# benabbouosama/DEEPL-Project

Hardware: AMD Instinct MI355X
Metric: images/sec train step, TransVAE-Large f16d32 256px bs256 (higher is better)
Workload: dtype bf16

## Files before the change

deepl-project_amd/csrc/wgrad_kx3.hip:

```cpp
#include "common.h"

#include <type_traits>

namespace {

struct Kx3Args {
    const bf16* x;
    const bf16* gy;
    float* dw;
    float* dbias;
    int M, h, w, c_in, ldx, c_out, ldo;
    int tiles_ci, chunk_px, hw_shift, w_shift, plain;
    int xcd_order, base, ny, accum;
    unsigned x_bytes;
};

template <int TW>
__device__ __forceinline__ int kx_swz(int c, int r) {
    if constexpr (TW % 128 == 0) {
        return (c & ~15) | ((c & 15) ^ ((r & 7) << 1));
    } else if constexpr (TW % 64 == 0) {
        return (c & ~7) | ((c & 7) ^ (((r >> 1) & 3) << 1));
    } else {
        static_assert(TW % 32 == 0, "tile width");
        return (c & ~3) | ((c & 3) ^ (((r >> 2) & 1) << 1));
    }
}

constexpr int kx_seg_stride(int seg) { return (seg + 2 + 7) / 8 * 8; }
constexpr int kx_x_pieces(int seg, int cx) { return ((64 / seg) * kx_seg_stride(seg) * cx + 63) / 64; }
constexpr int kx_stage_bytes(int tg, int tx, int seg) { return 64 * tg * 2 + kx_x_pieces(seg, tx / 8) * 1024; }

template <int TG, int TX, int NWM, int NWN, int RING, int VAR, int SEG, int TAPS = 3>
__global__ __launch_bounds__(512, 1) void wgrad_kx3_kernel(const Kx3Args p) {
    constexpr int NW = 8, BKP = 64;
    static_assert(NWM * NWN == NW, "8 waves");
    static_assert(SEG == 16 || SEG == 32 || SEG == 64, "segment = min(image width, 64)");
    static_assert(TAPS == 3 || (TAPS == 1 && SEG == 64), "one tap: 64 consecutive rows per K-step");
    constexpr int CG = TG / 8, CX = TX / 8;
    constexpr int NSEG = BKP / SEG, SS = TAPS == 1 ? 64 : kx_seg_stride(SEG);
    constexpr int G_PIECES = BKP * CG / 64;
    constexpr int X_PIECES = TAPS == 1 ? CX : kx_x_pieces(SEG, CX);
    static_assert(G_PIECES % NW == 0, "gy pieces divide over the waves");
    constexpr int G_IT = G_PIECES / NW, X_IT = (X_PIECES + NW - 1) / NW, P_IT = G_IT + X_IT;
    constexpr int XR = X_PIECES % NW;
    constexpr int G_BYTES = BKP * TG * 2, X_BYTES = X_PIECES * 1024;
    constexpr int KK_ROWS = SEG == 64 ? 32 : (32 / SEG) * SS, H_ROWS = SEG == 16 ? SS : 16;
    constexpr int X_REGION = RING * G_BYTES;
    static_assert(RING * (G_BYTES + X_BYTES) <= 160 * 1024, "LDS");
    constexpr int WTG = TG / NWM, WTX = TX / NWN, MF = WTG / 16, NF = WTX / 16;
    static_assert(WTG % 16 == 0 && WTX % 16 == 0, "wave tile");
    constexpr bool RD_SPLIT = VAR == 1 || VAR == 2 || VAR == 3;
    constexpr int LOOK = (VAR == 2 || VAR == 3) ? RING - 2 : RING - 1;
    constexpr int IT_SPLIT = VAR == 1 ? 0 : ((VAR == 2 || VAR == 4) ? G_IT : P_IT);
    static_assert(LOOK >= 2, "the wait at the end of load phase t covers K-step t + 1");

    extern __shared__ __attribute__((aligned(16))) char smem[];
    const int tid = threadIdx.x, lane = tid & 63;
    const int wave = __builtin_amdgcn_readfirstlane(tid >> 6);
    const int wm = wave / NWN, wn = wave % NWN;

    int bx, chunk_id;
    if (p.xcd_order) {
        const int lin = blockIdx.x;
        const int xcd = lin & 7, j = lin >> 3;
        bx = j % p.base;
        chunk_id = (j / p.base) * 8 + xcd;
        if (chunk_id >= p.ny) return;
    } else {
        bx = blockIdx.x;
        chunk_id = blockIdx.y;
    }
    const int ci_tile = bx % p.tiles_ci;
    bx /= p.tiles_ci;
    const int ky = TAPS == 3 ? bx % 3 : 0;
    const int co_tile = TAPS == 3 ? bx / 3 : bx;
    const int co0 = co_tile * TG, ci0 = ci_tile * TX;
    const int p_begin = chunk_id * p.chunk_px;
    const int p_end = min(p.M, p_begin + p.chunk_px);
    const int nsteps = (p_end - p_begin) / BKP;
    if (nsteps <= 0) return;
    const int w = p.w, hw = p.h * p.w;
    const int dty = TAPS == 3 ? ky - 1 : 0;

    int g_voff[G_IT];
#pragma unroll
    for (int it = 0; it < G_IT; ++it) {
        const int id = (it * NW + wave) * 64 + lane;
        const int r = id / CG, sl = id - r * CG;
        g_voff[it] = (r * p.ldo + co0 + kx_swz<TG>(sl, r) * 8) * 2;
    }
    int x_voff[X_IT], x_need[X_IT];
#pragma unroll
    for (int it = 0; it < X_IT; ++it) {
        const int id = (it * NW + wave) * 64 + lane;
        const int R = id / CX, sl = id - R * CX;
        const int sg = R / SS, o = R - sg * SS;
        const int need = TAPS == 1 ? 1 : (o == 0 ? 2 : (o == SEG + 1 ? 4 : (o > SEG + 1 ? 0 : 1)));
        x_need[it] = sg < NSEG ? need << (3 * sg) : 0;
        x_voff[it] = ((sg * SEG + o) * p.ldx + ci0 + kx_swz<TX>(sl, R) * 8) * 2;
    }
    const long long dshift = TAPS == 1 ? 0 : ((long long)dty * w - 1) * p.ldx;
    const bf16* xb = p.x + dshift;
    const unsigned xb_bytes = (unsigned)((long long)p.x_bytes - dshift * 2);
    const unsigned g_bytes = (unsigned)((long long)p_end * p.ldo * 2);

    auto x_have = [&](int step) {
        int have = 0;
        if constexpr (TAPS == 1) return 1;
#pragma unroll
        for (int sg = 0; sg < NSEG; ++sg) {
            const int pz = p_begin + step * BKP + sg * SEG;
            const int x0 = pz & (w - 1);
            const int uy = ((pz & (hw - 1)) >> p.w_shift) + dty;
            if ((unsigned)uy < (unsigned)p.h) have |= (1 | (x0 != 0 ? 2 : 0) | (x0 + SEG < w ? 4 : 0)) << (3 * sg);
        }
        return have;
    };
    auto issue_piece = [&](auto it_c, int step, int slot, int have) {
        constexpr int IT = decltype(it_c)::value;
        const int pz = p_begin + step * BKP;
        if constexpr (IT < G_IT) {
            buffer_load_lds16(p.gy, g_bytes, smem + slot * G_BYTES + (IT * NW + wave) * 1024, g_voff[IT], pz * p.ldo * 2);
        } else {
            constexpr int XI = IT - G_IT;
            if (XR != 0 && XI == X_IT - 1 && wave >= XR) return;
            buffer_load_lds16(xb, xb_bytes, smem + X_REGION + slot * X_BYTES + (XI * NW + wave) * 1024,
                              (x_need[XI] & have) ? x_voff[XI] : OOB_OFFSET, pz * p.ldx * 2);
        }
    };
    auto stage_issue = [&](int step, int slot) {
        const int have = x_have(step);
        static_for<P_IT>([&](auto it_c) { issue_piece(it_c, step, slot, have); });
    };

    const int g = lane >> 4, q = (lane >> 2) & 3, pp = lane & 3;
    const unsigned smem_addr = (unsigned)(uintptr_t)(__attribute__((address_space(3))) char*)smem;
    unsigned a_base[MF];
#pragma unroll
    for (int i = 0; i < MF; ++i) {
        const int r = 4 * g + q;
        const int col = wm * WTG + i * 16 + 4 * pp;
        a_base[i] = smem_addr + r * (TG * 2) + kx_swz<TG>(col >> 3, r) * 16 + (pp & 1) * 8;
    }
    unsigned b_base[TAPS][NF];
#pragma unroll
    for (int tp = 0; tp < TAPS; ++tp) {
        const int R = 4 * g + q + tp;
#pragma unroll
        for (int j = 0; j < NF; ++j) {
            const int col = wn * WTX + j * 16 + 4 * pp;
            b_base[tp][j] = smem_addr + X_REGION + R * (TX * 2) + kx_swz<TX>(col >> 3, R) * 16 + (pp & 1) * 8;
        }
    }
    constexpr int A_IN = 32 * TG * 2 + 16 * TG * 2, B_IN = (KK_ROWS + H_ROWS) * TX * 2;
    constexpr bool A_TWO = (RING - 1) * G_BYTES + A_IN >= 65536, B_TWO = (RING - 1) * X_BYTES + B_IN >= 65536;
    static_assert(!A_TWO || ((RING - 3) * G_BYTES + A_IN < 65536 && G_BYTES + A_IN < 65536), "gy slot offsets");
    static_assert(!B_TWO || ((RING - 3) * X_BYTES + B_IN < 65536 && X_BYTES + B_IN < 65536), "x slot offsets");
    unsigned a_base2[MF], b_base2[TAPS][NF];
#pragma unroll
    for (int i = 0; i < MF; ++i) a_base2[i] = a_base[i] + (A_TWO ? 2 * G_BYTES : 0);
#pragma unroll
    for (int tp = 0; tp < TAPS; ++tp)
#pragma unroll
        for (int j = 0; j < NF; ++j) b_base2[tp][j] = b_base[tp][j] + (B_TWO ? 2 * X_BYTES : 0);

    f32x4 acc[TAPS][MF][NF];
#pragma unroll
    for (int tp = 0; tp < TAPS; ++tp)
#pragma unroll
        for (int i = 0; i < MF; ++i)
#pragma unroll
            for (int j = 0; j < NF; ++j) acc[tp][i][j] = f32x4{0.f, 0.f, 0.f, 0.f};

    const bool do_bias = p.dbias != nullptr;
    const int nshare = TAPS * p.tiles_ci;
    int bias_ctr = ky * p.tiles_ci + ci_tile;
    bool own = false, own_prev = false;
    constexpr int NB = (MF + NWN - 1) / NWN;
    float bsum[NB];
#pragma unroll
    for (int k = 0; k < NB; ++k) bsum[k] = 0.f;

    auto join = [](bf16x4 lo, bf16x4 hi) { return bf16x8{lo[0], lo[1], lo[2], lo[3], hi[0], hi[1], hi[2], hi[3]}; };
    bf16x4 alo[2][MF], ahi[2][MF], blo[2][TAPS][NF], bhi[2][TAPS][NF];
    const int grp = wave >> 2;

    constexpr int NR = 2 * MF + 2 * TAPS * NF, NM = TAPS * MF * NF;
    auto frag_read = [&](auto kk_c, auto r_c, auto slot_c) {
        constexpr int KK = decltype(kk_c)::value, R = decltype(r_c)::value, SLOT = decltype(slot_c)::value;
        if constexpr (R < 2 * MF) {
            constexpr int i = R / 2, h = R % 2;
            constexpr int OFF = ((A_TWO && SLOT >= 2) ? (SLOT - 2) * G_BYTES : SLOT * G_BYTES) + KK * 32 * TG * 2 + h * 16 * TG * 2;
            const unsigned ab = (A_TWO && SLOT >= 2) ? a_base2[i] : a_base[i];
            if constexpr (h == 0) alo[KK][i] = lds_tr16_imm<OFF>(ab);
            else ahi[KK][i] = lds_tr16_imm<OFF>(ab);
        } else {
            constexpr int rr = R - 2 * MF, tp = rr / (2 * NF), j = (rr / 2) % NF, h = rr % 2;
            constexpr int OFF = ((B_TWO && SLOT >= 2) ? (SLOT - 2) * X_BYTES : SLOT * X_BYTES) + KK * KK_ROWS * TX * 2 + h * H_ROWS * TX * 2;
            const unsigned bb = (B_TWO && SLOT >= 2) ? b_base2[tp][j] : b_base[tp][j];
            if constexpr (h == 0) blo[KK][tp][j] = lds_tr16_imm<OFF>(bb);
            else bhi[KK][tp][j] = lds_tr16_imm<OFF>(bb);
        }
    };
    auto mfma_one = [&](auto kk_c, auto m_c) {
        constexpr int KK = decltype(kk_c)::value, M = decltype(m_c)::value;
        constexpr int i = M / (TAPS * NF), tp = (M / NF) % TAPS, j = M % NF;
        acc[tp][i][j] = __builtin_amdgcn_mfma_f32_16x16x32_bf16(join(alo[KK][i], ahi[KK][i]), join(blo[KK][tp][j], bhi[KK][tp][j]), acc[tp][i][j], 0, 0, 0);
    };
    auto bias_add = [&](auto kk_c) {
        constexpr int KK = decltype(kk_c)::value;
#pragma unroll
        for (int i = 0; i < MF; ++i)
            if (i % NWN == wn) {
                float a = 0.f;
#pragma unroll
                for (int e = 0; e < 4; ++e) a += (float)alo[KK][i][e] + (float)ahi[KK][i][e];
                bsum[i / NWN] += a;
            }
    };
    using I0 = std::integral_constant<int, 0>;
    using I1 = std::integral_constant<int, 1>;

#pragma unroll
    for (int st = 0; st < LOOK; ++st)
        if (st < nsteps) stage_issue(st, st);
    wait_vmcnt<0>();
    if (grp == 1) __builtin_amdgcn_s_barrier();

    auto step = [&](int t, auto slot_c) {
        constexpr int SLOT = decltype(slot_c)::value;
        constexpr int FILL = (SLOT + LOOK) % RING;
        const bool more = t + LOOK < nsteps;
        own_prev = own;
        own = do_bias && bias_ctr == 0;
        bias_ctr = bias_ctr == 0 ? nshare - 1 : bias_ctr - 1;
        __builtin_amdgcn_s_barrier();
        if constexpr (RD_SPLIT) {
            if (own_prev) bias_add(I1{});
            __builtin_amdgcn_sched_barrier(0);
        }
        static_for<NR>([&](auto r_c) { frag_read(I0{}, r_c, slot_c); });
        if constexpr (!RD_SPLIT) static_for<NR>([&](auto r_c) { frag_read(I1{}, r_c, slot_c); });
        __builtin_amdgcn_sched_barrier(0);
        const int have = more ? x_have(t + LOOK) : 0;
        if (more) static_for<IT_SPLIT>([&](auto it_c) { issue_piece(it_c, t + LOOK, FILL, have); });
        __builtin_amdgcn_sched_barrier(0);
        asm volatile("s_waitcnt lgkmcnt(0)" ::: "memory");
        __builtin_amdgcn_sched_barrier(0);
        if (own) {
            bias_add(I0{});
            if constexpr (!RD_SPLIT) bias_add(I1{});
        }
        {
            constexpr int NLG = IT_SPLIT < G_IT ? IT_SPLIT : G_IT;
            constexpr int NLX = IT_SPLIT > G_IT ? IT_SPLIT - G_IT : 0;
            constexpr int P_HI = G_IT + X_IT, P_LO = G_IT + X_IT - (XR != 0 ? 1 : 0);
            constexpr int L_HI = NLG + NLX, L_LO = NLG + NLX - ((XR != 0 && NLX == X_IT) ? 1 : 0);
            if (!more) wait_vmcnt<0>();
            else if (XR != 0 && wave < XR) wait_vmcnt<(LOOK - 2) * P_HI + L_HI>();
            else wait_vmcnt<(LOOK - 2) * P_LO + L_LO>();
        }
        __builtin_amdgcn_s_barrier();
        __builtin_amdgcn_s_setprio(1);
        if constexpr (!RD_SPLIT && IT_SPLIT == P_IT) {
            static_for<NM>([&](auto m_c) { mfma_one(I0{}, m_c); });
            static_for<NM>([&](auto m_c) { mfma_one(I1{}, m_c); });
        } else {
            constexpr int NP = P_IT - IT_SPLIT;
            static_for<NM>([&](auto m_c) {
                constexpr int M = decltype(m_c)::value;
                mfma_one(I0{}, m_c);
                __builtin_amdgcn_sched_barrier(0);
                if constexpr (RD_SPLIT) {
                    constexpr int r0 = M * NR / NM, r1 = (M + 1) * NR / NM;
                    static_for<r1 - r0>([&](auto d_c) { frag_read(I1{}, std::integral_constant<int, r0 + decltype(d_c)::value>{}, slot_c); });
                }
                if constexpr (NP > 0) {
                    static_for<NP>([&](auto k_c) {
                        constexpr int K = decltype(k_c)::value;
                        if constexpr ((2 * K + 1) * 2 * NM / (2 * NP) == M) {
                            if (more) issue_piece(std::integral_constant<int, IT_SPLIT + K>{}, t + LOOK, FILL, have);
                        }
                    });
                }
                __builtin_amdgcn_sched_barrier(0);
            });
            if constexpr (RD_SPLIT) {
                asm volatile("s_waitcnt lgkmcnt(0)" ::: "memory");
                __builtin_amdgcn_sched_barrier(0);
            }
            static_for<NM>([&](auto m_c) {
                constexpr int M = decltype(m_c)::value + NM;
                mfma_one(I1{}, m_c);
                if constexpr (NP > 0) {
                    __builtin_amdgcn_sched_barrier(0);
                    static_for<NP>([&](auto k_c) {
                        constexpr int K = decltype(k_c)::value;
                        if constexpr ((2 * K + 1) * 2 * NM / (2 * NP) == M) {
                            if (more) issue_piece(std::integral_constant<int, IT_SPLIT + K>{}, t + LOOK, FILL, have);
                        }
                    });
                    __builtin_amdgcn_sched_barrier(0);
                }
            });
        }
        __builtin_amdgcn_s_setprio(0);
        __builtin_amdgcn_sched_barrier(0);
    };

    for (int t = 0; t < nsteps; t += RING) {
        step(t, std::integral_constant<int, 0>{});
        if (t + 1 < nsteps) step(t + 1, std::integral_constant<int, 1>{});
        if (t + 2 < nsteps) step(t + 2, std::integral_constant<int, 2 % RING>{});
        if constexpr (RING == 4) {
            if (t + 3 < nsteps) step(t + 3, std::integral_constant<int, 3 % RING>{});
        }
    }
    if constexpr (RD_SPLIT) {
        if (own) bias_add(I1{});
    }
    if (grp == 0) __builtin_amdgcn_s_barrier();

    const size_t ldw = (size_t)(TAPS * TAPS) * p.c_in;
#pragma unroll
    for (int i = 0; i < MF; ++i) {
#pragma unroll
        for (int r = 0; r < 4; ++r) {
            const int co = co0 + wm * WTG + i * 16 + g * 4 + r;
#pragma unroll
            for (int tp = 0; tp < TAPS; ++tp) {
                float* rowp = p.dw + (size_t)co * ldw + (size_t)(ky * TAPS + tp) * p.c_in;
#pragma unroll
                for (int j = 0; j < NF; ++j) {
                    const int ci = ci0 + wn * WTX + j * 16 + (lane & 15);
                    if (p.plain && !p.accum) rowp[ci] = acc[tp][i][j][r];
                    else if (p.plain) rowp[ci] += acc[tp][i][j][r];
                    else atomicAdd(rowp + ci, acc[tp][i][j][r]);
                }
            }
        }
    }
    if (do_bias) {
#pragma unroll
        for (int i = 0; i < MF; ++i)
            if (i % NWN == wn) {
                float v = bsum[i / NWN];
                v += __shfl_xor(v, 16, 64);
                v += __shfl_xor(v, 32, 64);
                const int co = co0 + wm * WTG + i * 16 + (lane & 15);
                if (lane < 16) atomicAdd(p.dbias + co, v);
            }
    }
}

int g_kx3_ring = 0;
int g_kx3_var = -1;
int g_kx3_blocks = 0;

template <int TG, int TX, int NWM, int NWN, int RING, int VAR, int SEG, int TAPS = 3>
int kx3_launch_v(const Kx3Args& a, dim3 grid, hipStream_t s) {
    constexpr int BYTES = RING * (TAPS == 1 ? 64 * (TG + TX) * 2 : kx_stage_bytes(TG, TX, SEG));
    static_assert(BYTES <= 160 * 1024, "LDS");
    static TvPerDeviceOnce attr_once;
    if (attr_once.first()) {
        (void)hipFuncSetAttribute((const void*)wgrad_kx3_kernel<TG, TX, NWM, NWN, RING, VAR, SEG, TAPS>, hipFuncAttributeMaxDynamicSharedMemorySize, BYTES);
    }
    hipLaunchKernelGGL((wgrad_kx3_kernel<TG, TX, NWM, NWN, RING, VAR, SEG, TAPS>), grid, dim3(512), BYTES, s, a);
    return 0;
}

template <int TG, int TX, int NWM, int NWN, int RING, int SEG, int TAPS = 3>
int kx3_launch_r(Kx3Args a, hipStream_t s, bool plan_only) {
    const int tiles_co = a.c_out / TG;
    a.tiles_ci = a.c_in / TX;
    const long long base = (long long)tiles_co * TAPS * a.tiles_ci;
    const double t_px = 2.0 * TG * TX * TAPS * 256.0 / 1200e12;
    const double tile_bytes = 4.0 * TG * TX * TAPS;
    long long split = 1;
    bool xcd = false;
    double best = 1e30;
    const long long smax = a.M / 512 > 0 ? a.M / 512 : 1;
    if (g_kx3_blocks) {
        split = (g_kx3_blocks + base - 1) / base;
        xcd = base <= 32 && split >= 8;
    } else {
        for (long long sp = 1; sp <= smax && sp <= 4096; ++sp) {
            const double rounds = (double)((long long)((base * sp + 255) / 256));
            const double t = rounds * ((double)a.M / sp) * t_px + (sp > 1 ? base * sp * tile_bytes / 1.3e12 : 0.0);
            if (t < best) { best = t; split = sp; xcd = false; }
        }
        if (base <= 32) {
            for (long long sp = 8; sp <= smax && sp <= 4096; sp += 8) {
                const double rounds = (double)((long long)((base * (sp / 8) + 31) / 32));
                const double t = rounds * ((double)a.M / sp) * (t_px * 0.85) + base * sp * tile_bytes / 1.3e12;
                if (t < best) { best = t; split = sp; xcd = true; }
            }
        }
    }
    long long chunk = (a.M + split - 1) / split;
    if (chunk < 512) chunk = 512;
    chunk = (chunk + 63) / 64 * 64;
    a.chunk_px = (int)chunk;
    const int ny = (int)((a.M + chunk - 1) / chunk);
    a.plain = (ny == 1) ? 1 : 0;
    if (plan_only) return 100 + a.plain;
    a.base = (int)base;
    a.ny = ny;
    a.xcd_order = (ny > 1 && xcd) ? 1 : 0;
    dim3 grid((unsigned)base, (unsigned)ny);
    if (a.xcd_order) grid = dim3((unsigned)(8 * base * ((ny + 7) / 8)), 1);
    if constexpr (TAPS == 1) {
        if (g_kx3_var == 0) return kx3_launch_v<TG, TX, NWM, NWN, RING, 0, SEG, 1>(a, grid, s);
        return kx3_launch_v<TG, TX, NWM, NWN, RING, 4, SEG, 1>(a, grid, s);
    } else if constexpr (RING == 4 && SEG == 64) {
        switch (g_kx3_var < 0 ? 4 : g_kx3_var) {
            case 1: return kx3_launch_v<TG, TX, NWM, NWN, RING, 1, SEG>(a, grid, s);
            case 2: return kx3_launch_v<TG, TX, NWM, NWN, RING, 2, SEG>(a, grid, s);
            case 3: return kx3_launch_v<TG, TX, NWM, NWN, RING, 3, SEG>(a, grid, s);
            case 4: return kx3_launch_v<TG, TX, NWM, NWN, RING, 4, SEG>(a, grid, s);
            default: break;
        }
    }
    if (g_kx3_var != 0) return kx3_launch_v<TG, TX, NWM, NWN, RING, 4, SEG>(a, grid, s);
    return kx3_launch_v<TG, TX, NWM, NWN, RING, 0, SEG>(a, grid, s);
}

template <int TG, int TX, int NWM, int NWN, int SEG>
int kx3_launch_s(const Kx3Args& a, hipStream_t s, bool plan_only) {
    if constexpr (4 * kx_stage_bytes(TG, TX, SEG) <= 160 * 1024) {
        if (g_kx3_ring != 3) return kx3_launch_r<TG, TX, NWM, NWN, 4, SEG>(a, s, plan_only);
    }
    return kx3_launch_r<TG, TX, NWM, NWN, 3, SEG>(a, s, plan_only);
}

template <int TG, int TX, int NWM, int NWN>
int kx3_launch(const Kx3Args& a, hipStream_t s, bool plan_only) {
    if (a.w >= 64) return kx3_launch_s<TG, TX, NWM, NWN, 64>(a, s, plan_only);
    if (a.w == 32) return kx3_launch_s<TG, TX, NWM, NWN, 32>(a, s, plan_only);
    return kx3_launch_s<TG, TX, NWM, NWN, 16>(a, s, plan_only);
}

}

extern "C" int tv_set_wgrad_kx3(int enable, int ring, int blocks);
int g_kx3_enable = 2;
int g_kx3_prefer128 = 0;
extern "C" int tv_set_wgrad_kx3(int enable, int ring, int blocks) {
    g_kx3_enable = enable;
    g_kx3_ring = ring % 10;
    g_kx3_var = ring >= 10 ? ring / 10 : (ring == 0 ? -1 : 0);
    g_kx3_blocks = blocks % 100000;
    g_kx3_prefer128 = blocks / 100000;
    return 0;
}

int tv_wgrad_kx3_try(const tv_conv_desc* d, const void* x, const void* gy, float* dw, float* dbias, hipStream_t s, bool plan_only, int accum) {
    if (!g_kx3_enable) return -1;
    auto log2_exact = [](int v) { int sh = 0; while ((1 << sh) < v) ++sh; return ((1 << sh) == v) ? sh : -1; };
    if (d->kh == 1 && d->kw == 1) {
        const long long Ml = (long long)d->batch * d->h_out * d->w_out;
        const bool ok = g_kx3_enable % 10 >= 2 && d->stride == 1 && d->pad == 0 && d->up_shift == 0 && d->dil_mask == 0 && d->h_in == d->h_out &&
                        d->w_in == d->w_out && Ml % 64 == 0 && Ml * d->ldx * 2 < (1ll << 31) && Ml * d->ldo * 2 < (1ll << 31) &&
                        d->c_out % 192 == 0 && d->c_in % 192 == 0;
        if (!ok) return -1;
        Kx3Args a;
        a.x = (const bf16*)x; a.gy = (const bf16*)gy; a.dw = dw; a.dbias = dbias;
        a.M = (int)Ml; a.h = 1; a.w = 64; a.c_in = d->c_in; a.ldx = d->ldx; a.c_out = d->c_out; a.ldo = d->ldo;
        a.tiles_ci = 1; a.chunk_px = 0; a.hw_shift = 6; a.w_shift = 6; a.plain = 0;
        a.xcd_order = 0; a.base = 1; a.ny = 1; a.accum = accum;
        a.x_bytes = (unsigned)(Ml * d->ldx * 2);
        const int tsel = g_kx3_enable / 10;
        if (tsel == 1 && d->c_out % 256 == 0 && d->c_in % 128 == 0) return kx3_launch_r<256, 128, 4, 2, 3, 64, 1>(a, s, plan_only);
        if (tsel == 2 && d->c_out % 128 == 0 && d->c_in % 256 == 0) return kx3_launch_r<128, 256, 2, 4, 3, 64, 1>(a, s, plan_only);
        return kx3_launch_r<192, 192, 4, 2, 3, 64, 1>(a, s, plan_only);
    }
    const int wsh = log2_exact(d->w_out), hwsh = log2_exact(d->h_out * d->w_out);
    const long long M = (long long)d->batch * d->h_out * d->w_out;
    const long long xbytes = M * d->ldx * 2, gbytes = M * d->ldo * 2;
    const bool geo = d->kh == 3 && d->kw == 3 && d->stride == 1 && d->pad == 1 && d->up_shift == 0 && d->dil_mask == 0 &&
                     d->h_in == d->h_out && d->w_in == d->w_out && wsh >= 4 && hwsh >= 6 &&
                     xbytes + (long long)(d->w_in + 1) * d->ldx * 2 < (1ll << 31) && gbytes < (1ll << 31);
    if (!geo) return -1;
    const bool t192 = d->c_out % 192 == 0 && d->c_in % 96 == 0;
    const bool t128 = d->c_out % 128 == 0 && d->c_in % 128 == 0;
    if (!t192 && !t128) return -1;
    Kx3Args a;
    a.x = (const bf16*)x; a.gy = (const bf16*)gy; a.dw = dw; a.dbias = dbias;
    a.M = (int)M; a.h = d->h_out; a.w = d->w_out; a.c_in = d->c_in; a.ldx = d->ldx; a.c_out = d->c_out; a.ldo = d->ldo;
    a.tiles_ci = 1; a.chunk_px = 0; a.hw_shift = hwsh; a.w_shift = wsh; a.plain = 0;
    a.xcd_order = 0; a.base = 1; a.ny = 1; a.accum = accum;
    a.x_bytes = (unsigned)xbytes;
    if (t192 && !(t128 && g_kx3_prefer128 != 2)) return kx3_launch<192, 96, 4, 2>(a, s, plan_only);
    return kx3_launch<128, 128, 2, 4>(a, s, plan_only);
}
```

Before: 160.6.

## Add wide 384x192 tiles with 32-row K-steps for 1x1 weight-gradient kernel

After: 161.5 (median of 6 runs). Within noise of the previous version (+0.6%).

```diff
diff --git a/deepl-project_amd/csrc/wgrad_kx3.hip b/deepl-project_amd/csrc/wgrad_kx3.hip
--- a/deepl-project_amd/csrc/wgrad_kx3.hip
+++ b/deepl-project_amd/csrc/wgrad_kx3.hip
@@ -31,18 +31,19 @@
 constexpr int kx_x_pieces(int seg, int cx) { return ((64 / seg) * kx_seg_stride(seg) * cx + 63) / 64; }
 constexpr int kx_stage_bytes(int tg, int tx, int seg) { return 64 * tg * 2 + kx_x_pieces(seg, tx / 8) * 1024; }
 
-template <int TG, int TX, int NWM, int NWN, int RING, int VAR, int SEG, int TAPS = 3>
+template <int TG, int TX, int NWM, int NWN, int RING, int VAR, int SEG, int TAPS = 3, int KH = 2>
 __global__ __launch_bounds__(512, 1) void wgrad_kx3_kernel(const Kx3Args p) {
-    constexpr int NW = 8, BKP = 64;
+    constexpr int NW = 8, BKP = 32 * KH;
     static_assert(NWM * NWN == NW, "8 waves");
+    static_assert(KH == 2 || (KH == 1 && TAPS == 1 && (VAR == 0 || VAR == 4)), "32-row K-steps: one tap, every read in the load phase");
     static_assert(SEG == 16 || SEG == 32 || SEG == 64, "segment = min(image width, 64)");
     static_assert(TAPS == 3 || (TAPS == 1 && SEG == 64), "one tap: 64 consecutive rows per K-step");
     constexpr int CG = TG / 8, CX = TX / 8;
-    constexpr int NSEG = BKP / SEG, SS = TAPS == 1 ? 64 : kx_seg_stride(SEG);
+    constexpr int NSEG = TAPS == 1 ? 1 : BKP / SEG, SS = TAPS == 1 ? 64 : kx_seg_stride(SEG);
     constexpr int G_PIECES = BKP * CG / 64;
-    constexpr int X_PIECES = TAPS == 1 ? CX : kx_x_pieces(SEG, CX);
-    static_assert(G_PIECES % NW == 0, "gy pieces divide over the waves");
-    constexpr int G_IT = G_PIECES / NW, X_IT = (X_PIECES + NW - 1) / NW, P_IT = G_IT + X_IT;
+    constexpr int X_PIECES = TAPS == 1 ? BKP * CX / 64 : kx_x_pieces(SEG, CX);
+    constexpr int G_IT = (G_PIECES + NW - 1) / NW, X_IT = (X_PIECES + NW - 1) / NW, P_IT = G_IT + X_IT;
+    constexpr int GR = G_PIECES % NW;
     constexpr int XR = X_PIECES % NW;
     constexpr int G_BYTES = BKP * TG * 2, X_BYTES = X_PIECES * 1024;
     constexpr int KK_ROWS = SEG == 64 ? 32 : (32 / SEG) * SS, H_ROWS = SEG == 16 ? SS : 16;
@@ -121,12 +122,13 @@
         constexpr int IT = decltype(it_c)::value;
         const int pz = p_begin + step * BKP;
         if constexpr (IT < G_IT) {
+            if (GR != 0 && IT == G_IT - 1 && wave >= GR) return;
             buffer_load_lds16(p.gy, g_bytes, smem + slot * G_BYTES + (IT * NW + wave) * 1024, g_voff[IT], pz * p.ldo * 2);
         } else {
             constexpr int XI = IT - G_IT;
             if (XR != 0 && XI == X_IT - 1 && wave >= XR) return;
             buffer_load_lds16(xb, xb_bytes, smem + X_REGION + slot * X_BYTES + (XI * NW + wave) * 1024,
-                              (x_need[XI] & have) ? x_voff[XI] : OOB_OFFSET, pz * p.ldx * 2);
+                              (TAPS == 1 || (x_need[XI] & have)) ? x_voff[XI] : OOB_OFFSET, pz * p.ldx * 2);
         }
     };
     auto stage_issue = [&](int step, int slot) {
@@ -153,7 +155,7 @@
             b_base[tp][j] = smem_addr + X_REGION + R * (TX * 2) + kx_swz<TX>(col >> 3, R) * 16 + (pp & 1) * 8;
         }
     }
-    constexpr int A_IN = 32 * TG * 2 + 16 * TG * 2, B_IN = (KK_ROWS + H_ROWS) * TX * 2;
+    constexpr int A_IN = (KH - 1) * 32 * TG * 2 + 16 * TG * 2, B_IN = ((KH - 1) * KK_ROWS + H_ROWS) * TX * 2;
     constexpr bool A_TWO = (RING - 1) * G_BYTES + A_IN >= 65536, B_TWO = (RING - 1) * X_BYTES + B_IN >= 65536;
     static_assert(!A_TWO || ((RING - 3) * G_BYTES + A_IN < 65536 && G_BYTES + A_IN < 65536), "gy slot offsets");
     static_assert(!B_TWO || ((RING - 3) * X_BYTES + B_IN < 65536 && X_BYTES + B_IN < 65536), "x slot offsets");
@@ -183,7 +185,7 @@
     for (int k = 0; k < NB; ++k) bsum[k] = 0.f;
 
     auto join = [](bf16x4 lo, bf16x4 hi) { return bf16x8{lo[0], lo[1], lo[2], lo[3], hi[0], hi[1], hi[2], hi[3]}; };
-    bf16x4 alo[2][MF], ahi[2][MF], blo[2][TAPS][NF], bhi[2][TAPS][NF];
+    bf16x4 alo[KH][MF], ahi[KH][MF], blo[KH][TAPS][NF], bhi[KH][TAPS][NF];
     const int grp = wave >> 2;
 
     constexpr int NR = 2 * MF + 2 * TAPS * NF, NM = TAPS * MF * NF;
@@ -241,7 +243,7 @@
             __builtin_amdgcn_sched_barrier(0);
         }
         static_for<NR>([&](auto r_c) { frag_read(I0{}, r_c, slot_c); });
-        if constexpr (!RD_SPLIT) static_for<NR>([&](auto r_c) { frag_read(I1{}, r_c, slot_c); });
+        if constexpr (!RD_SPLIT && KH == 2) static_for<NR>([&](auto r_c) { frag_read(I1{}, r_c, slot_c); });
         __builtin_amdgcn_sched_barrier(0);
         const int have = more ? x_have(t + LOOK) : 0;
         if (more) static_for<IT_SPLIT>([&](auto it_c) { issue_piece(it_c, t + LOOK, FILL, have); });
@@ -250,22 +252,26 @@
         __builtin_amdgcn_sched_barrier(0);
         if (own) {
             bias_add(I0{});
-            if constexpr (!RD_SPLIT) bias_add(I1{});
+            if constexpr (!RD_SPLIT && KH == 2) bias_add(I1{});
         }
         {
             constexpr int NLG = IT_SPLIT < G_IT ? IT_SPLIT : G_IT;
             constexpr int NLX = IT_SPLIT > G_IT ? IT_SPLIT - G_IT : 0;
-            constexpr int P_HI = G_IT + X_IT, P_LO = G_IT + X_IT - (XR != 0 ? 1 : 0);
-            constexpr int L_HI = NLG + NLX, L_LO = NLG + NLX - ((XR != 0 && NLX == X_IT) ? 1 : 0);
+            constexpr int GS = GR != 0 ? 1 : 0, XS = XR != 0 ? 1 : 0;
+            constexpr int LGS = (GS && NLG == G_IT) ? 1 : 0, LXS = (XS && NLX == X_IT) ? 1 : 0;
+            constexpr int P_ALL = G_IT + X_IT, L_ALL = NLG + NLX;
+            const bool gs = GR != 0 && wave >= GR, xs = XR != 0 && wave >= XR;
             if (!more) wait_vmcnt<0>();
-            else if (XR != 0 && wave < XR) wait_vmcnt<(LOOK - 2) * P_HI + L_HI>();
-            else wait_vmcnt<(LOOK - 2) * P_LO + L_LO>();
+            else if (gs && xs) wait_vmcnt<(LOOK - 2) * (P_ALL - GS - XS) + L_ALL - LGS - LXS>();
+            else if (gs) wait_vmcnt<(LOOK - 2) * (P_ALL - GS) + L_ALL - LGS>();
+            else if (xs) wait_vmcnt<(LOOK - 2) * (P_ALL - XS) + L_ALL - LXS>();
+            else wait_vmcnt<(LOOK - 2) * P_ALL + L_ALL>();
         }
         __builtin_amdgcn_s_barrier();
         __builtin_amdgcn_s_setprio(1);
         if constexpr (!RD_SPLIT && IT_SPLIT == P_IT) {
             static_for<NM>([&](auto m_c) { mfma_one(I0{}, m_c); });
-            static_for<NM>([&](auto m_c) { mfma_one(I1{}, m_c); });
+            if constexpr (KH == 2) static_for<NM>([&](auto m_c) { mfma_one(I1{}, m_c); });
         } else {
             constexpr int NP = P_IT - IT_SPLIT;
             static_for<NM>([&](auto m_c) {
@@ -279,7 +285,7 @@
                 if constexpr (NP > 0) {
                     static_for<NP>([&](auto k_c) {
                         constexpr int K = decltype(k_c)::value;
-                        if constexpr ((2 * K + 1) * 2 * NM / (2 * NP) == M) {
+                        if constexpr ((2 * K + 1) * KH * NM / (2 * NP) == M) {
                             if (more) issue_piece(std::integral_constant<int, IT_SPLIT + K>{}, t + LOOK, FILL, have);
                         }
                     });
@@ -290,14 +296,14 @@
                 asm volatile("s_waitcnt lgkmcnt(0)" ::: "memory");
                 __builtin_amdgcn_sched_barrier(0);
             }
-            static_for<NM>([&](auto m_c) {
+            if constexpr (KH == 2) static_for<NM>([&](auto m_c) {
                 constexpr int M = decltype(m_c)::value + NM;
                 mfma_one(I1{}, m_c);
                 if constexpr (NP > 0) {
                     __builtin_amdgcn_sched_barrier(0);
                     static_for<NP>([&](auto k_c) {
                         constexpr int K = decltype(k_c)::value;
-                        if constexpr ((2 * K + 1) * 2 * NM / (2 * NP) == M) {
+                        if constexpr ((2 * K + 1) * KH * NM / (2 * NP) == M) {
                             if (more) issue_piece(std::integral_constant<int, IT_SPLIT + K>{}, t + LOOK, FILL, have);
                         }
                     });
@@ -358,19 +364,19 @@
 int g_kx3_var = -1;
 int g_kx3_blocks = 0;
 
-template <int TG, int TX, int NWM, int NWN, int RING, int VAR, int SEG, int TAPS = 3>
+template <int TG, int TX, int NWM, int NWN, int RING, int VAR, int SEG, int TAPS = 3, int KH = 2>
 int kx3_launch_v(const Kx3Args& a, dim3 grid, hipStream_t s) {
-    constexpr int BYTES = RING * (TAPS == 1 ? 64 * (TG + TX) * 2 : kx_stage_bytes(TG, TX, SEG));
+    constexpr int BYTES = RING * (TAPS == 1 ? 32 * KH * (TG + TX) * 2 : kx_stage_bytes(TG, TX, SEG));
     static_assert(BYTES <= 160 * 1024, "LDS");
     static TvPerDeviceOnce attr_once;
     if (attr_once.first()) {
-        (void)hipFuncSetAttribute((const void*)wgrad_kx3_kernel<TG, TX, NWM, NWN, RING, VAR, SEG, TAPS>, hipFuncAttributeMaxDynamicSharedMemorySize, BYTES);
-    }
-    hipLaunchKernelGGL((wgrad_kx3_kernel<TG, TX, NWM, NWN, RING, VAR, SEG, TAPS>), grid, dim3(512), BYTES, s, a);
+        (void)hipFuncSetAttribute((const void*)wgrad_kx3_kernel<TG, TX, NWM, NWN, RING, VAR, SEG, TAPS, KH>, hipFuncAttributeMaxDynamicSharedMemorySize, BYTES);
+    }
+    hipLaunchKernelGGL((wgrad_kx3_kernel<TG, TX, NWM, NWN, RING, VAR, SEG, TAPS, KH>), grid, dim3(512), BYTES, s, a);
     return 0;
 }
 
-template <int TG, int TX, int NWM, int NWN, int RING, int SEG, int TAPS = 3>
+template <int TG, int TX, int NWM, int NWN, int RING, int SEG, int TAPS = 3, int KH = 2>
 int kx3_launch_r(Kx3Args a, hipStream_t s, bool plan_only) {
     const int tiles_co = a.c_out / TG;
     a.tiles_ci = a.c_in / TX;
@@ -410,7 +416,9 @@
     a.xcd_order = (ny > 1 && xcd) ? 1 : 0;
     dim3 grid((unsigned)base, (unsigned)ny);
     if (a.xcd_order) grid = dim3((unsigned)(8 * base * ((ny + 7) / 8)), 1);
-    if constexpr (TAPS == 1) {
+    if constexpr (TAPS == 1 && KH == 1) {
+        return kx3_launch_v<TG, TX, NWM, NWN, RING, 4, SEG, 1, 1>(a, grid, s);
+    } else if constexpr (TAPS == 1) {
         if (g_kx3_var == 0) return kx3_launch_v<TG, TX, NWM, NWN, RING, 0, SEG, 1>(a, grid, s);
         return kx3_launch_v<TG, TX, NWM, NWN, RING, 4, SEG, 1>(a, grid, s);
     } else if constexpr (RING == 4 && SEG == 64) {
@@ -422,8 +430,10 @@
             default: break;
         }
     }
-    if (g_kx3_var != 0) return kx3_launch_v<TG, TX, NWM, NWN, RING, 4, SEG>(a, grid, s);
-    return kx3_launch_v<TG, TX, NWM, NWN, RING, 0, SEG>(a, grid, s);
+    if constexpr (TAPS == 3) {
+        if (g_kx3_var != 0) return kx3_launch_v<TG, TX, NWM, NWN, RING, 4, SEG>(a, grid, s);
+        return kx3_launch_v<TG, TX, NWM, NWN, RING, 0, SEG>(a, grid, s);
+    }
 }
 
 template <int TG, int TX, int NWM, int NWN, int SEG>
@@ -439,6 +449,15 @@
     if (a.w >= 64) return kx3_launch_s<TG, TX, NWM, NWN, 64>(a, s, plan_only);
     if (a.w == 32) return kx3_launch_s<TG, TX, NWM, NWN, 32>(a, s, plan_only);
     return kx3_launch_s<TG, TX, NWM, NWN, 16>(a, s, plan_only);
+}
+
+int kx3_wide_tile(int c_out, int c_in) {
+    static const struct { int c_out, c_in, tile; } tab[] = {
+        {6144, 1536, 4}, {3072, 768, 4}, {768, 3072, 4}, {2304, 768, 3}, {384, 1536, 4}, {1152, 384, 4},
+    };
+    for (const auto& e : tab)
+        if (e.c_out == c_out && e.c_in == c_in) return e.tile;
+    return 0;
 }
 
 }
@@ -473,6 +492,10 @@
         const int tsel = g_kx3_enable / 10;
         if (tsel == 1 && d->c_out % 256 == 0 && d->c_in % 128 == 0) return kx3_launch_r<256, 128, 4, 2, 3, 64, 1>(a, s, plan_only);
         if (tsel == 2 && d->c_out % 128 == 0 && d->c_in % 256 == 0) return kx3_launch_r<128, 256, 2, 4, 3, 64, 1>(a, s, plan_only);
+        const bool w_ci = d->c_in % 384 == 0, w_co = d->c_out % 384 == 0;
+        const int wide = tsel == 0 ? kx3_wide_tile(d->c_out, d->c_in) : tsel;
+        if (wide == 3 && w_ci) return kx3_launch_r<192, 384, 2, 4, 4, 64, 1, 1>(a, s, plan_only);
+        if (wide == 4 && w_co) return kx3_launch_r<384, 192, 4, 2, 4, 64, 1, 1>(a, s, plan_only);
         return kx3_launch_r<192, 192, 4, 2, 3, 64, 1>(a, s, plan_only);
     }
     const int wsh = log2_exact(d->w_out), hwsh = log2_exact(d->h_out * d->w_out);
```
